# laurentbartholdi/SpaSM.jl

Measured on AMD Instinct MI355X. Metric: Schur nnz reduced/sec (GF(p) echelonize), 1Mx1M CSR, higher is better.
Workload: dtype int32 (GF(p) balanced residues); 1 GPU; BASELINE config 3: 1000000x1000000 CSR, 20 nnz/row, p=65521, seed 0x5A5A0003, Schur round 0; rows_per_gpu=1000000, npiv=169473, nnz_out=522630694, parallelism=single GPU

## Files before the change

spasm.jl_amd/csrc/engine.hip:

```cpp
#include "common.hpp"
#include "kernels.hpp"
#include "stream.hpp"
#include "wlevel.hpp"
#include "greedy.hpp"
#include "dense.hpp"
#include "spmv.hpp"
#include "spgemm.hpp"
#include "trsolve.hpp"
#include "batch.hpp"
#include <cstring>
#include <rocprim/device/device_scan.hpp>
#include <rocprim/device/device_radix_sort.hpp>
#include <vector>
#include <memory>
#include <stdexcept>
#include <type_traits>
#include <algorithm>
#include <cstring>
#include <cstdlib>
#include <condition_variable>
#include <mutex>
#include <thread>
#include <atomic>
#include <string>
// ... 94 lines not shown
}

template <int LOGT, int TPR, int WPB, int MAXR, bool SMALL, int MINW = 1> void init_scatter(size_t lds)
{
    static bool attr_done[kMaxDev] = {false};
    bool &done = attr_done[current_device()];
    if (!done) {
        HIPCHK(hipFuncSetAttribute((const void *)k_scatter<LOGT, TPR, WPB, MAXR, SMALL, MINW>, hipFuncAttributeMaxDynamicSharedMemorySize, (int)lds));
        done = true;
    }
}
template <int LOGT, int TPR, int WPB, int MAXR, bool SMALL, int MINW = 1> void launch_scatter(const ScatterArgs &a, int grid, size_t lds, hipStream_t s)
{
    init_scatter<LOGT, TPR, WPB, MAXR, SMALL, MINW>(lds);
    if (grid <= 0) return;
    hipLaunchKernelGGL((k_scatter<LOGT, TPR, WPB, MAXR, SMALL, MINW>), dim3(grid), dim3(WPB * 64), lds, s, a);
    HIPCHK(hipGetLastError());
}

template <bool SMALL> void launch_scatter_class(int cls, const ScatterArgs &a, int grid, size_t lds, hipStream_t s)
{
    switch (cls) {
    case 0: launch_scatter<8, 64, 4, 1, SMALL>(a, grid, lds, s); break;
    case 1: launch_scatter<9, 64, 4, 2, SMALL>(a, grid, lds, s); break;
    case 2: launch_scatter<10, 64, 4, 4, SMALL, 4>(a, grid, lds, s); break;
    case 3: launch_scatter<11, 128, 2, 4, SMALL, 4>(a, grid, lds, s); break;
    case 4: launch_scatter<12, 256, 4, 4, SMALL, 4>(a, grid, lds, s); break;
    case 5: launch_scatter<13, 256, 4, 5, SMALL>(a, grid, lds, s); break;
    case 6: if (SMALL) launch_scatter<14, 256, 4, 5, true>(a, grid, lds, s); break;
    default: break;
    }
}

template <int LOGT, int TPR, int WPB, int B, bool SMALL, int MINW = 1, int EPL = 1, int QX = 0, bool BLOOM = false> void launch_wstream(const StreamArgs &a, int nrows, int num_cu, size_t lds, hipStream_t s)
{
    static int per_cu_dev[kMaxDev] = {0};
    int &per_cu = per_cu_dev[current_device()];
    if (!per_cu) {
        HIPCHK(hipFuncSetAttribute((const void *)k_wstream<LOGT, TPR, WPB, B, SMALL, MINW, EPL, QX, BLOOM>, hipFuncAttributeMaxDynamicSharedMemorySize, (int)lds));
        int nb = 0;
        HIPCHK(hipOccupancyMaxActiveBlocksPerMultiprocessor(&nb, (const void *)k_wstream<LOGT, TPR, WPB, B, SMALL, MINW, EPL, QX, BLOOM>, WPB * 64, lds));
        per_cu = std::max(nb, 1);
    }
    if (nrows <= 0) return;
    const int rows_per_block = TPR == 64 ? WPB : 1;
    const int grid = std::max(1, std::min((nrows + rows_per_block - 1) / rows_per_block, num_cu * per_cu));
    hipLaunchKernelGGL((k_wstream<LOGT, TPR, WPB, B, SMALL, MINW, EPL, QX, BLOOM>), dim3(grid), dim3(WPB * 64), lds, s, a);
    HIPCHK(hipGetLastError());
}

inline bool stream_bloom()
{
    const char *e = getenv("SPASM_AMD_BLOOM");
    return e && atoi(e) != 0;
}
inline int stream_chunk_log()
{
    const char *e = getenv("SPASM_AMD_CHUNK");
    return e && atoi(e) == 128 ? 7 : 6;
}

const int kNumStreamClasses = 7;
inline int stream_logt(int c) { return 8 + c; }
inline int stream_tpr(int c) { return c <= 2 ? 64 : (c == 3 ? 128 : 256); }
inline int stream_wpb(int c) { return c == 3 ? 2 : 4; }
template <bool SMALL> void launch_stream_class(int cls, const StreamArgs &a, int nrows, int num_cu, size_t lds, hipStream_t s, int chunk_log = 6)
{
    if (chunk_log == 7) {
        switch (cls) {
        case 0: launch_wstream<8, 64, 4, 2, SMALL, 1, 2>(a, nrows, num_cu, lds, s); break;
        case 1: launch_wstream<9, 64, 4, 4, SMALL, 1, 2>(a, nrows, num_cu, lds, s); break;
        case 2: launch_wstream<10, 64, 4, 4, SMALL, 1, 2>(a, nrows, num_cu, lds, s); break;
        case 3: launch_wstream<11, 128, 2, 4, SMALL, 1, 2>(a, nrows, num_cu, lds, s); break;
        case 4: launch_wstream<12, 256, 4, 4, SMALL, 1, 2>(a, nrows, num_cu, lds, s); break;
        case 5: launch_wstream<13, 256, 4, 4, SMALL, 1, 2>(a, nrows, num_cu, lds, s); break;
        case 6: launch_wstream<14, 256, 4, 4, SMALL, 1, 2>(a, nrows, num_cu, lds, s); break;
        default: break;
        }
        return;
    }
    if (stream_bloom()) {
        switch (cls) {
        case 0: launch_wstream<8, 64, 4, 4, SMALL, 1, 1, 0, true>(a, nrows, num_cu, lds, s); break;
        case 1: launch_wstream<9, 64, 4, 8, SMALL, 1, 1, 0, true>(a, nrows, num_cu, lds, s); break;
        case 2: launch_wstream<10, 64, 4, 8, SMALL, 1, 1, 0, true>(a, nrows, num_cu, lds, s); break;
        case 3: launch_wstream<11, 128, 2, 8, SMALL, 1, 1, 0, true>(a, nrows, num_cu, lds, s); break;
        case 4: launch_wstream<12, 256, 4, 8, SMALL, 1, 1, 0, true>(a, nrows, num_cu, lds, s); break;
        case 5: launch_wstream<13, 256, 4, 8, SMALL, 1, 1, 0, true>(a, nrows, num_cu, lds, s); break;
        case 6: launch_wstream<14, 256, 4, 8, SMALL, 1, 1, 0, true>(a, nrows, num_cu, lds, s); break;
        default: break;
        }
        return;
    }
    switch (cls) {
    case 0: launch_wstream<8, 64, 4, 4, SMALL>(a, nrows, num_cu, lds, s); break;
    case 1: launch_wstream<9, 64, 4, 8, SMALL>(a, nrows, num_cu, lds, s); break;
    case 2: launch_wstream<10, 64, 4, 8, SMALL>(a, nrows, num_cu, lds, s); break;
    case 3: launch_wstream<11, 128, 2, 8, SMALL>(a, nrows, num_cu, lds, s); break;
    case 4: launch_wstream<12, 256, 4, 8, SMALL>(a, nrows, num_cu, lds, s); break;
    case 5: launch_wstream<13, 256, 4, 8, SMALL>(a, nrows, num_cu, lds, s); break;
    case 6: launch_wstream<14, 256, 4, 8, SMALL>(a, nrows, num_cu, lds, s); break;
    default: break;
    }
}

struct Round {
    ZpField F;
    int m = 0;
    int num_cu = 256;
    hipStream_t stream = nullptr;
    Scanner scan;

    DevBuf<u64d> best;
    DevBuf<int> colflag, colscan, qinv_r, pivrow, pivcol, is_piv, rowflag, rowscan, np_rows;
    int npiv = 0, nnp = 0;
    DevBuf<i64d> ulen, uoff;
    i64 utotal = 0;
    DevBuf<int2> Ufull, UPP, UPN;
    DevBuf<UHdr> uhdr;
    bool use_uinv = false;
    DevMat E;
    DevBuf<int2> UinvPool;
    DevBuf<i64d> UinvStart, ubound;
    DevBuf<int> UinvLen;
    DevBuf<int4> colinfo;
    DevBuf<unsigned> pbits;
    DevBuf<i64d> rstart;
    DevBuf<int> rlen;
    i64 uinv_nnz = 0;
    DevBuf<int4> Lpool;
    DevBuf<int> Lidx;
    bool want_idx = false;
    DevBuf<int> sflag;
    DevBuf<int2> fixbuf;
    DevBuf<int> fixcnt;
    bool use_stream = true;
    int chunk_log = 6;
    bool use_w = false;
    bool force_lists = false;
    DevBuf<int4> wcol;
    DevBuf<int2> wrow;
    DevBuf<int> wreject_list;
    i64 wtotal = 0;
    i64 wcap = 0;
    i64 w_entries = 0, w_long_rows = 0;
    i64 own_base = 0, wbase = 0;
    i64 own_total = 0;
    DevBuf<u64d> own_ctr;
    DevBuf<u64d> wstate, wblk;
    DevBuf<int> wmid_list, wbig_list, wbig_count;
    std::vector<int> wbig_at;
    bool want_w_row_stats = false;
    DevBuf<WLevRec> lev_recs;
    DevBuf<unsigned> lev0_sz, lev0_off;
    DevBuf<u64d> lev0_ent;
    i64 lev0_total = 0, lev0_entries = 0;
    int wave_per_cu_blocks = 0;
    DevBuf<int> lev, lev_keys, lev_iota, lev_order, lev_start_d, lev_flag;
    DevBuf<unsigned char> sort_tmp;
    std::vector<int> lev_start;
    int depth = -1;
    bool quiet_rejects = false;
    DevBuf<u64d> pool_ctr;
    int npool_active = NPOOL;
    u64d region_cap = 0;
    DevBuf<i64d> Lstart, bound, sstart;
    DevBuf<int> Llen, overflow_list, overflow2_list, fail_list;
    DevBuf<long long> pmask;
    int big_blocks = 0, big_npiv = -1;
    DevBuf<int> xdense;
// ... 835 lines not shown
        rstart.ensure((size_t)nrows + 1);
        rlen.ensure((size_t)nrows + 1);
        hipLaunchKernelGGL(k_gather_rows, dim3(cdiv(nrows, 256)), dim3(256), 0, stream, nrows, rows, M.start.p, M.len.p, rstart.p, rlen.p);
        HIPCHK(hipGetLastError());
        if (wmode) {
            wreject_list.ensure((size_t)nrows + 1);
            WPlanArgs wp;
            wp.nrows = nrows;
            wp.rstart = rstart.p;
            wp.rlen = rlen.p;
            wp.ent = M.ent.p;
            wp.pbits = pbits.p;
            wp.wcol = wcol.p;
            wp.Lpool = Lpool.p;
            wp.lpool_cap = region_cap;
            wp.pool_ctr = pool_ctr.p;
            wp.npool = npool_active;
            wp.upn = UPN.p;
            wp.own_base = (unsigned)own_base;
            wp.own_cap = (u64d)own_total / (u64d)npool_active;
            wp.own_ctr = own_ctr.p;
            wp.Lstart = Lstart.p;
            wp.Llen = Llen.p;
            wp.bound = bound.p;
            wp.pmask = pmask.p;
            wp.sflag = sflag.p;
            wp.free_cols = free_cols;
            wp.max_bound = (int)kClasses[kNumStreamClasses - 1].cap;
            wp.wave_row_bound = (int)kClasses[2].cap;
            wp.overflow_list = wreject_list.p;
            wp.overflow_count = &ctr.p->wplan_reject;
            wp.ctr = ctr.p;
            wp.F = F;
            chunk_log = stream_chunk_log();
            wp.chunk_log = chunk_log;
            constexpr int TEAM = 16, TPB = 256;
            hipLaunchKernelGGL((k_wplan<TEAM, TPB>), dim3(std::min(cdiv((i64)nrows * TEAM, TPB), num_cu * 16)), dim3(TPB), 0, stream, wp);
            HIPCHK(hipGetLastError());
            if (!use_uinv) {
                if (!quiet_rejects) launch_chain(a, nrows, true, wreject_list.p, &ctr.p->wplan_reject);
                return;
            }
        }
        CombineArgs c;
        c.nrows = nrows;
        c.self_idx = self_idx;
        c.rstart = rstart.p;
        c.rlen = rlen.p;
        c.ent = M.ent.p;
        c.colinfo = colinfo.p;
        c.pbits = pbits.p;
        c.uhdr = uhdr.p;
        c.UinvPool = UinvPool.p;
        c.Lpool = Lpool.p;
        c.Lidx = want_idx ? Lidx.p : nullptr;
        c.sflag = nullptr;
        c.lpool_cap = region_cap;
        c.pool_ctr = pool_ctr.p;
        c.npool = npool_active;
        c.Lstart = Lstart.p;
        c.Llen = Llen.p;
        c.bound = bound.p;
        c.pmask = pmask.p;
        c.free_cols = free_cols;
        c.retry = wmode ? wreject_list.p : nullptr;
        c.retry_count = wmode ? &ctr.p->wplan_reject : nullptr;
        c.overflow_list = overflow2_list.p;
        c.overflow_count = &ctr.p->combine_overflow;
        c.ctr = ctr.p;
        {
// ... 110 lines not shown
                HIPCHK(hipStreamCreateWithFlags(&twin_s[t], hipStreamNonBlocking));
                HIPCHK(hipEventCreateWithFlags(&twin_ev[t], hipEventDisableTiming));
            }
    }
    void ensure_big_scatter(hipStream_t s)
    {
        if (bigsc_m == m) return;
        const i64 per = std::max<i64>((i64)m, 1) * 13;
        bigsc_blocks = (int)std::max<i64>(1, std::min<i64>((i64)num_cu * 8, ((i64)2 << 30) / per));
        bigsc_m = m;
        const size_t nw = ((size_t)std::max(m, 1) + 31) / 32;
        sc_xdense.alloc((size_t)bigsc_blocks * (size_t)std::max(m, 1));
        sc_bitmap.alloc((size_t)bigsc_blocks * nw);
        sc_touched.alloc((size_t)bigsc_blocks * (size_t)std::max(m, 1));
        sc_xdense.zero(s);
        sc_bitmap.zero(s);
    }
    void warm_scatter()
    {
        ensure_streams();
        ensure_big_scatter(stream);
        ScatterArgs a;
        memset(&a, 0, sizeof a);
        StreamArgs sa;
        memset(&sa, 0, sizeof sa);
        const int nhash = F.small ? kNumHashClasses : kNumHashClasses - 1;
        for (int c = 0; c < nhash; c++) {
            const size_t lds = scatter_lds_bytes(kClasses[c], F.small);
            if (F.small) launch_scatter_class<true>(c, a, 0, lds, stream);
            else launch_scatter_class<false>(c, a, 0, lds, stream);
        }
        for (int c = 0; c < std::min(nhash, kNumStreamClasses); c++) {
            const size_t lds = stream_lds_bytes(stream_logt(c), stream_tpr(c), stream_wpb(c));
            if (F.small) launch_stream_class<true>(c, sa, 0, num_cu, lds, stream, stream_chunk_log());
            else launch_stream_class<false>(c, sa, 0, num_cu, lds, stream, stream_chunk_log());
        }
    }

    void run_scatter(const DevMat &M, const int *rows, int nrows)
    {
        const int4 *recs = Lpool.p;
        S.n = nrows;
        S.m = m;
        nlaunch = 0;
        if (nrows == 0) return;
        int nhash = F.small ? kNumHashClasses : kNumHashClasses - 1;
        const bool streaming = use_w && !force_lists && !want_idx;
        BinArgs b;
        b.nrows = nrows;
        b.bound = bound.p;
        b.Llen = Llen.p;
        for (int c = 0; c < NCLASS; c++) b.cap[c] = -1;
        for (int c = 0; c < nhash; c++) b.cap[c] = kClasses[c].cap;
        b.lazy_terms = zp_lazy_terms(F);
        b.class_count = class_count.p;
        b.class_list = class_list.p;
        b.rows = rows;
        b.start = M.start.p;
        b.len = M.len.p;
        b.orig = M.orig.p;
        b.Lstart = Lstart.p;
        b.sstart = sstart.p;
        b.pmask = pmask.p;
        b.sflag = sflag.p;
        b.stream_classes = streaming ? std::min(nhash, kNumStreamClasses) : 0;
        b.Sorig = S.orig.p;
        b.fixcnt = fixcnt.p;
        b.desc = class_desc.p;
// ... 40 lines not shown
        const bool use_side = !class_timing && (nhash > first_side || streaming);
        if (use_side) {
            ensure_streams();
            HIPCHK(hipEventRecord(ev_fork, stream));
            HIPCHK(hipStreamWaitEvent(side, ev_fork, 0));
        }
        auto mark = [&](int cls_id, hipStream_t s) {
            if (!class_timing || nlaunch >= NCLASS) return;
            HIPCHK(hipEventRecord(ev_cls[nlaunch], s));
            launch_cls[nlaunch++] = cls_id;
        };
        auto launch_class = [&](int c, hipStream_t s) {
            mark(c, s);
            a.cls = c;
            a.class_count = class_count.p + c;
            a.desc = class_desc.p + (size_t)c * nrows;
            const size_t lds = scatter_lds_bytes(kClasses[c], F.small);
            int per_cu = (int)std::min<size_t>(32 / kClasses[c].wpb, (160 * 1024) / lds);
            if (per_cu < 1) per_cu = 1;
            const int rows_per_block = kClasses[c].tpr == 64 ? kClasses[c].wpb : 1;
            const int grid = std::max(1, std::min(cdiv(nrows, rows_per_block), num_cu * per_cu));
            if (F.small) launch_scatter_class<true>(c, a, grid, lds, s);
            else launch_scatter_class<false>(c, a, grid, lds, s);
        };
        auto launch_stream_cls = [&](int c, hipStream_t s) {
            if (!streaming || c >= kNumStreamClasses) return;
            mark(NSTREAM0 + c, s);
            sa.cls = NSTREAM0 + c;
            sa.class_count = class_count.p + NSTREAM0 + c;
            sa.desc = class_desc.p + (size_t)(NSTREAM0 + c) * nrows;
            sa.redo_count = class_count.p + c;
            sa.redo_desc = class_desc.p + (size_t)c * nrows;
            const size_t lds = stream_lds_bytes(stream_logt(c), stream_tpr(c), stream_wpb(c));
            if (F.small) launch_stream_class<true>(c, sa, nrows, num_cu, lds, s, chunk_log);
            else launch_stream_class<false>(c, sa, nrows, num_cu, lds, s, chunk_log);
        };
        auto launch_stream_fix = [&](hipStream_t s) {
            if (!streaming) return;
            mark(NCLASS - 1, s);
            StreamFixArgs fa;
            fa.nrows = nrows;
            fa.fixcnt = fixcnt.p;
            fa.fixbuf = fixbuf.p;
            fa.sstart = sstart.p;
            fa.Sent = S.ent.p;
            fa.Slen = S.len.p;
            fa.Slead = S.lead.p;
            fa.ctr = ctr.p;
            fa.F = F;
            hipLaunchKernelGGL(k_stream_fix, dim3(cdiv(nrows, 64)), dim3(256), 0, s, fa);
            HIPCHK(hipGetLastError());
        };
        auto launch_big = [&](hipStream_t s) {
            ensure_big_scatter(s);
            mark(NHASHMAX - 1, s);
            BigScatterArgs bb;
            bb.s = a;
            bb.s.cls = NHASHMAX - 1;
            bb.s.class_count = class_count.p + (NHASHMAX - 1);
            bb.s.desc = class_desc.p + (size_t)(NHASHMAX - 1) * nrows;
            bb.m = std::max(m, 1);
            bb.nwords = (std::max(m, 1) + 31) / 32;
            bb.xdense = sc_xdense.p;
            bb.bitmap = sc_bitmap.p;
            bb.touched = sc_touched.p;
            hipLaunchKernelGGL(k_scatter_big, dim3(bigsc_blocks), dim3(256), 0, s, bb);
            HIPCHK(hipGetLastError());
        };
// ... 5716 lines not shown
```

spasm.jl_amd/csrc/stream.hpp:

```cpp
#pragma once
#include "kernels.hpp"

struct StreamArgs {
    const int *class_count;
    const RowDesc *desc;
    const int2 *ent;
    const int *qinv_r;
    const int2 *UPN;
    const int4 *Lpool;
    int2 *Sent;
    int *Slen;
    int *Slead;
    RoundCounters *ctr;
    int cls;
    int *redo_count;
    RowDesc *redo_desc;
    int2 *fixbuf;
    int *fixcnt;
    u64d *stamps;
    int dbg;
    ZpField F;
};

constexpr int SLCAP = 64;
// ... 186 lines not shown
}


struct WPlanArgs {
    int nrows;
    const i64d *rstart;
    const int *rlen;
    const int2 *ent;
    const unsigned *pbits;
    const int4 *wcol;
    int4 *Lpool;
    u64d lpool_cap;
    u64d *pool_ctr;
    int npool;
    int2 *upn;
    unsigned own_base;
    u64d own_cap;
    u64d *own_ctr;
    i64d *Lstart;
    int *Llen;
    i64d *bound;
    long long *pmask;
    int *sflag;
    int free_cols;
    int max_bound;
    int wave_row_bound;
    int *overflow_list;
    int *overflow_count;
    RoundCounters *ctr;
    ZpField F;
    int chunk_log;
};

template <int TEAM, int TPB>
__global__ __launch_bounds__(TPB) void k_wplan(WPlanArgs a)
{
    constexpr int TEAMS = TPB / TEAM;
    constexpr u64d RBLK = 64, OBLK = 256;
    const int tl = threadIdx.x % TEAM;
    const int team = threadIdx.x / TEAM;
    const ZpField F = a.F;
    const int CL = a.chunk_log, CH = 1 << CL;
    u64d rpos = 0, rend = 0, opos = 0, oend = 0;
    auto take = [&](u64d &pos, u64d &end, u64d need, u64d blk, u64d *ctr, u64d cap) -> u64d {
        if (pos + need > end) {
            const u64d n = need > blk ? need : blk;
            u64d b = 0;
            if (tl == 0) b = pool_alloc(ctr, cap, n, a.npool);
            b = __shfl(b, 0, TEAM);
            if (b == ~0ull) return ~0ull;
            pos = b;
            end = b + n;
        }
        const u64d r = pos;
        pos += need;
        return r;
    };
    auto is_piv = [&](int c) -> bool { return (a.pbits[(unsigned)c >> 5] >> (c & 31)) & 1u; };
    const i64d first = (i64d)blockIdx.x * TEAMS + team, stride = (i64d)gridDim.x * TEAMS;
    i64d st_n = 0;
    int ln_n = 0;
    int2 ea_n = make_int2(0, 0), eb_n = make_int2(0, 0);
    if (first < a.nrows) {
        st_n = a.rstart[first];
        ln_n = a.rlen[first];
        if (tl < ln_n) ea_n = a.ent[st_n + tl];
        if (tl + TEAM < ln_n) eb_n = a.ent[st_n + tl + TEAM];
    }
    for (i64d t64 = first; t64 < a.nrows; t64 += stride) {
        const int t = (int)t64;
        const i64d st = st_n;
        const int ln = ln_n;
        const int2 ea = ea_n, eb = eb_n;
        if (t64 + stride < a.nrows) {
            st_n = a.rstart[t64 + stride];
            ln_n = a.rlen[t64 + stride];
            ea_n = make_int2(0, 0);
            eb_n = make_int2(0, 0);
            if (tl < ln_n) ea_n = a.ent[st_n + tl];
            if (tl + TEAM < ln_n) eb_n = a.ent[st_n + tl + TEAM];
        }
        int C = 0, nN = 0;
        bool zero_own = false;
        u64d pm = 0;
        int4 ci_a = make_int4(-1, 0, 0, 0), ci_b = ci_a;
        bool pa = false, pb = false;
        for (int k0 = 0; k0 < ln; k0 += TEAM) {
            const int k = k0 + tl;
            const bool valid = k < ln;
            int2 e = k0 == 0 ? ea : (k0 == TEAM ? eb : make_int2(0, 0));
            if (k0 >= 2 * TEAM && valid) e = a.ent[st + k];
            const bool isP = valid && is_piv(e.x);
            int4 ci = make_int4(-1, 0, 0, 0);
            if (isP) ci = a.wcol[e.x];
            if (k0 == 0) { ci_a = ci; pa = isP; }
            if (k0 == TEAM) { ci_b = ci; pb = isP; }
            zero_own |= valid && (e.y == 0 || (isP && ci.y < 0));
            const u64d mP = team_ballot<TEAM>(isP);
            if (k0 < 64) pm |= mP << (k0 & 63);
            int tot;
            (void)team_incl_scan<TEAM>(isP ? (ci.y + CH - 1) >> CL : 0, tot);
            C += tot;
            nN += __popcll(team_ballot<TEAM>(valid && !isP));
        }
        const bool anyzero = team_ballot<TEAM>(zero_own) != 0;
        const int own_chunks = (nN + CH - 1) >> CL;
        const int R = C + own_chunks;
        const u64d base = take(rpos, rend, (u64d)R, RBLK, a.pool_ctr, a.lpool_cap);
        const u64d obase = base == ~0ull ? ~0ull : take(opos, oend, (u64d)nN, OBLK, a.own_ctr, a.own_cap);
        i64d run = nN;
        int w = own_chunks, no = 0;
        const bool room = base != ~0ull && obase != ~0ull;
        for (int k0 = 0; k0 < ln && room; k0 += TEAM) {
            const int k = k0 + tl;
            const bool valid = k < ln;
            int2 e = k0 == 0 ? ea : (k0 == TEAM ? eb : make_int2(0, 0));
            if (k0 >= 2 * TEAM && valid) e = a.ent[st + k];
            bool isP = k0 == 0 ? pa : (k0 == TEAM ? pb : false);
            int4 ci = k0 == 0 ? ci_a : (k0 == TEAM ? ci_b : make_int4(-1, 0, 0, 0));
            if (k0 >= 2 * TEAM) {
                isP = valid && is_piv(e.x);
                if (isP) ci = a.wcol[e.x];
            }
            const u64d mN = team_ballot<TEAM>(valid && !isP);
            if (valid && !isP) a.upn[(size_t)a.own_base + obase + no + __popcll(mN & ((1ull << tl) - 1ull))] = e;
            no += __popcll(mN);
            const int len = isP ? ci.y : 0;
            const int nch = (len + CH - 1) >> CL;
            int tot, ctot;
            const int incl = team_incl_scan<TEAM>(len, tot);
            const int cincl = team_incl_scan<TEAM>(nch, ctot);
            const int nm = zp_neg(F, e.y);
            i64d pre = run + incl - len;
            int4 *out = a.Lpool + base + w + (cincl - nch);
            for (int q = 0; q < nch; q++) {
                const int clen = min(CH, len - CH * q);
                const unsigned px = (pre < 0x8000 ? (unsigned)pre : 0x7fffu) << 16 | (unsigned)clen;
                out[q] = make_int4((int)px, nm, (int)((unsigned)ci.z + (unsigned)CH * (unsigned)q), clen);
                pre += clen;
            }
            w += ctot;
            run += tot;
        }
        if (room)
            for (int q = tl; q < own_chunks; q += TEAM) {
                const int clen = min(CH, nN - CH * q);
                a.Lpool[base + q] = make_int4((int)(((unsigned)(CH * q) << 16) | (unsigned)clen), -1, (int)(a.own_base + (unsigned)obase + (unsigned)CH * (unsigned)q), clen);
            }
        if (tl == 0) {
            if (base == ~0ull) {
                atomicAdd(&ctr_shard(a.ctr)->lpool_overflow, 1);
                a.Llen[t] = 0; a.Lstart[t] = 0; a.bound[t] = 0;
            } else {
                const i64d bound = run;
                const bool ok = room && bound <= (i64d)a.free_cols && bound <= (i64d)a.max_bound && !anyzero && R <= (bound <= (i64d)a.wave_row_bound ? 64 : 256);
                if (ok) {
                    a.Lstart[t] = (i64d)base;
                    a.Llen[t] = R;
                    a.bound[t] = bound;
                    a.pmask[t] = ln <= 32 ? (long long)pm : -1;
                    a.sflag[t] = 1;
                } else {
                    a.Llen[t] = -1; a.Lstart[t] = 0; a.bound[t] = 0;
                    a.overflow_list[atomicAdd(a.overflow_count, 1)] = t;
                }
            }
        }
    }
}

typedef int v4i32s __attribute__((ext_vector_type(4)));
template <int LOGT, int TPR, int WPB, int D, bool SMALL, int MINW, int EPL = 1, int QX = 0, bool BLOOM = false>
__global__ __launch_bounds__(WPB * 64, MINW) void k_wstream(StreamArgs a)
{
    static_assert(EPL == 1 || EPL == 2, "one or two entries per lane");
    static_assert(!(BLOOM && EPL == 2), "the filter is built for one entry per lane");
    constexpr bool WAVE_ROW = (TPR == 64);
    static_assert(WAVE_ROW || TPR == WPB * 64, "a row is owned by one wave or by the whole workgroup");
    constexpr int NW = WAVE_ROW ? 1 : WPB;
    constexpr int FCAP = SFIX;
    constexpr size_t TABB = (size_t)4 * StreamTabs<LOGT>::WORDS, MISCB = 64, FIXB = (size_t)FCAP * 8;
    constexpr size_t SLOT = stream_row_bytes(LOGT);
    extern __shared__ __attribute__((aligned(16))) unsigned char s_raw[];
    const int tid = threadIdx.x;
    const int lane = tid & 63;
    const int wave = __builtin_amdgcn_readfirstlane(tid >> 6);
    const int rtid = WAVE_ROW ? lane : tid;
    const int rw = WAVE_ROW ? 0 : wave;
    unsigned char *base = s_raw + (WAVE_ROW ? (size_t)wave * SLOT : 0);
    StreamTabs<LOGT> tb;
    tb.bind(base);
    int *misc = (int *)(base + TABB);
    int2 *fix = (int2 *)(base + TABB + MISCB);
    int4 *lst = (int4 *)(base + TABB + MISCB + FIXB);
    const ZpField F = a.F;

    const int count = *a.class_count;
    if ((WAVE_ROW ? (int)blockIdx.x * WPB : (int)blockIdx.x) >= count) return;
    for (int s = rtid * 4; s < StreamTabs<LOGT>::WORDS; s += TPR * 4) *(int4 *)(tb.t1 + s) = make_int4(0, 0, 0, 0);
    if (rtid < 16) misc[rtid] = (rtid & 7) >= 4 ? INT_MAX : 0;
    __syncthreads();

    const int first = WAVE_ROW ? (int)blockIdx.x * WPB + wave : (int)blockIdx.x;
    const int stride = WAVE_ROW ? (int)gridDim.x * WPB : (int)gridDim.x;
    u64d c_nnz = 0, c_ent = 0, c_seg = 0;
    int c_rows = 0, c_redo = 0;
    int par = 0;

    RowDesc d, dn, dnn;
    int4 rec, rec_n;
    auto load_rec = [&](const RowDesc &dd) { return a.Lpool[dd.l_start + min(rw + lane * NW, max(dd.llen - 1, 0))]; };
    d = stream_desc_unpack(stream_desc_load(a.desc + min(first, count - 1)));
    dn = stream_desc_unpack(stream_desc_load(a.desc + min(first + stride, count - 1)));
    dnn = stream_desc_unpack(stream_desc_load(a.desc + min(first + 2 * stride, count - 1)));
    rec = load_rec(d);
    rec_n = load_rec(dn);
    typedef typename std::conditional<EPL == 2, int4, int2>::type ring_t;
    ring_t ring[D];
    auto ring_load = [&](unsigned off, int clen) -> ring_t {
        if constexpr (EPL == 2) {
            const v4i32s v = *(const v4i32s *)(a.UPN + (size_t)off + (unsigned)min(2 * lane, clen - 1));
            return make_int4(v.x, v.y, v.z, v.w);
        } else {
            return a.UPN[(size_t)off + (unsigned)min(lane, clen - 1)];
        }
    };
    auto request = [&](const int4 &rc, int nmine, bool live) {
#pragma unroll
        for (int j = 0; j < D; j++) {
            const int g = min(j, max(nmine - 1, 0));
            const bool have = live && nmine > 0;
            const unsigned off = have ? (unsigned)__builtin_amdgcn_readlane(rc.z, g) : 0u;
            const int clen = have ? __builtin_amdgcn_readlane(rc.w, g) : 1;
            if constexpr (EPL == 1) {
                if (SCATTER_DBG(a, 8)) { ring[j] = make_int2(lane + 4096 * j, 1); continue; }
            }
            ring[j] = ring_load(off, clen);
        }
    };
    auto chunks_of = [&](int ll) { return ll > rw ? (ll - rw + NW - 1) / NW : 0; };
    request(rec, chunks_of(d.llen), first < count);

#ifdef SPASM_STAMPS
    u64d st_sum[NSTAMP] = {0, 0, 0, 0, 0, 0, 0, 0};
    u64d st_last = stamp_now();
#endif
    for (int w = first; w < count; w += stride) {
        const int d3_reg = stream_desc_load(a.desc + min(w + 3 * stride, count - 1));
        const int4 rec_nn = load_rec(dnn);
        const int ll = d.llen, E = d.bound, t_cur = d.t;
        int *const mrow = misc + par * 8;
        unsigned char *const rowp = (unsigned char *)(a.Sent + d.s_start);
        int mylead = INT_MAX;
        const int my_chunks = chunks_of(ll);
        STAMP(0);
        constexpr int Q = QX ? QX : (EPL == 2 ? (D >= 2 ? 2 : 1) : (D >= 4 ? 4 : D));
        constexpr int NE = Q * EPL;
        static_assert(D % Q == 0, "whole groups of slots");
        auto do_group = [&](const ring_t (&e)[Q], int g0, int nthere) {
            int cc[NE], vv[NE], pp[NE], cl[Q];
            bool there[NE];
            unsigned oo[NE], left[NE];
#pragma unroll
            for (int q = 0; q < Q; q++) {
                const int g = min(g0 + q, max(my_chunks - 1, 0));
                const int rx = __builtin_amdgcn_readlane(rec.x, g);
                const int nmul = -__builtin_amdgcn_readlane(rec.y, g);
                cl[q] = rx & 0xffff;
                if constexpr (EPL == 2) {
                    const int i0 = min(2 * lane, cl[q] - 1);
                    const bool second = 2 * lane + 1 < cl[q];
                    cc[2 * q] = e[q].x;
                    vv[2 * q] = stream_mul<SMALL>(F, nmul, e[q].y);
                    pp[2 * q] = (int)((unsigned)rx >> 16) + i0 + 1;
                    cc[2 * q + 1] = second ? e[q].z : e[q].x;
                    vv[2 * q + 1] = second ? stream_mul<SMALL>(F, nmul, e[q].w) : vv[2 * q];
                    pp[2 * q + 1] = pp[2 * q] + (second ? 1 : 0);
                    there[2 * q] = 2 * lane < cl[q];
                    there[2 * q + 1] = second;
                } else {
                    cc[q] = e[q].x;
                    vv[q] = stream_mul<SMALL>(F, nmul, e[q].y);
                    pp[q] = (int)((unsigned)rx >> 16) + min(lane, cl[q] - 1) + 1;
                    there[q] = lane < cl[q];
                }
            }
#pragma unroll
            for (int k = 0; k < NE; k++) { oo[k] = 0; left[k] = 0; }
            auto store_chunk = [&](int q) {
                if constexpr (EPL == 2) {
                    if (cl[q] == 128) {
                        v4i32s v;
                        v.x = cc[2 * q]; v.y = vv[2 * q]; v.z = cc[2 * q + 1]; v.w = vv[2 * q + 1];
                        __builtin_nontemporal_store(v, (v4i32s *)(rowp + ((unsigned)(pp[2 * q] - 1) << 3)));
                    } else {
                        __builtin_nontemporal_store(((long long)(unsigned)vv[2 * q] << 32) | (unsigned)cc[2 * q], (long long *)(rowp + ((unsigned)(pp[2 * q] - 1) << 3)));
                        __builtin_nontemporal_store(((long long)(unsigned)vv[2 * q + 1] << 32) | (unsigned)cc[2 * q + 1], (long long *)(rowp + ((unsigned)(pp[2 * q + 1] - 1) << 3)));
                    }
// ... 30 lines not shown
                }
                return;
            }
            if (nthere >= Q) {
#pragma unroll
                for (int q = 0; q < Q; q++)
                    if (!SCATTER_DBG(a, 1)) store_chunk(q);
                    else if constexpr (EPL == 2) mylead = min(mylead, min(cc[2 * q], cc[2 * q + 1]));
                    else mylead = min(mylead, cc[q]);
                if (!SCATTER_DBG(a, 2)) stream_insert_n<LOGT, NE>(tb, cc, pp, oo, left);
            } else {
#pragma unroll
                for (int q = 0; q < Q; q++)
                    if (q < nthere) {
                        store_chunk(q);
                        int c1[EPL], p1[EPL];
                        unsigned o1[EPL], l1[EPL];
#pragma unroll
                        for (int u = 0; u < EPL; u++) { c1[u] = cc[EPL * q + u]; p1[u] = pp[EPL * q + u]; }
                        stream_insert_n<LOGT, EPL>(tb, c1, p1, o1, l1);
#pragma unroll
                        for (int u = 0; u < EPL; u++) { oo[EPL * q + u] = o1[u]; left[EPL * q + u] = l1[u]; }
                    }
            }
            unsigned any = 0;
#pragma unroll
            for (int k = 0; k < NE; k++) any |= left[k];
            if (__ballot(any != 0) != 0) {
#pragma unroll
                for (int k = 0; k < NE; k++)
                    stream_report(stream_outcome(left[k]), oo[k], k / EPL < nthere && there[k], cc[k], vv[k], pp[k], mrow, fix, FCAP, lst);
            }
        };
        const int next_chunks = chunks_of(dn.llen);
        const bool next_live = w + stride < count;
#pragma unroll
        for (int j0 = 0; j0 < D; j0 += Q) {
            if (j0 < my_chunks) {
                ring_t e[Q];
#pragma unroll
                for (int q = 0; q < Q; q++) e[q] = ring[j0 + q];
                do_group(e, j0, my_chunks - j0);
            }
        }
        if (my_chunks > D) {
            for (int g0 = D; g0 < my_chunks; g0 += Q) {
                ring_t e[Q];
#pragma unroll
                for (int q = 0; q < Q; q++) {
                    const int g = min(g0 + q, my_chunks - 1);
                    e[q] = ring_load((unsigned)__builtin_amdgcn_readlane(rec.z, g), __builtin_amdgcn_readlane(rec.w, g));
                }
                do_group(e, g0, my_chunks - g0);
            }
        }
        STAMP(1);
        request(rec_n, next_chunks, next_live);
        STAMP(2);
        mylead = wave_min_i32(mylead);
        int lead_out = mylead;
        if (!WAVE_ROW) {
            if (lane == 0) mrow[4 + wave] = mylead;
            lds_barrier();
#pragma unroll
            for (int w2 = 0; w2 < WPB; w2++) lead_out = min(lead_out, mrow[4 + w2]);
        }
        if constexpr (BLOOM) {
            const int nsus = __builtin_amdgcn_readfirstlane(((lds_vint *)mrow)[1]);
            if (nsus != 0 && nsus <= SLCAP) {
                auto scan = [&](bool owners) {
                    for (int g0 = 0; g0 < my_chunks; g0 += 8) {
                        int2 e[8];
                        int ps[8], nm[8];
                        bool ok[8];
#pragma unroll
                        for (int u = 0; u < 8; u++) {
                            const int g = min(g0 + u, my_chunks - 1);
                            const int clen = __builtin_amdgcn_readlane(rec.w, g);
                            e[u] = a.UPN[(size_t)(unsigned)__builtin_amdgcn_readlane(rec.z, g) + (unsigned)min(lane, clen - 1)];
                            ps[u] = (int)((unsigned)__builtin_amdgcn_readlane(rec.x, g) >> 16) + lane;
                            nm[u] = -__builtin_amdgcn_readlane(rec.y, g);
                            ok[u] = g0 + u < my_chunks && lane < clen;
                        }
                        for (int i = 0; i < nsus; i++) {
                            const int4 sp = lst[i];
                            if (owners && !(sp.w != INT_MAX && sp.w > sp.z)) continue;
#pragma unroll
                            for (int u = 0; u < 8; u++) {
                                if (ok[u] && e[u].x == sp.x && ps[u] != sp.z) {
                                    if (!owners) atomicMin(&lst[i].w, ps[u]);
// ... 27 lines not shown
            const int nlist = __builtin_amdgcn_readfirstlane(((lds_vint *)mrow)[1]);
            redo = nlist > SLCAP;
            if (!BLOOM && nlist != 0 && !redo) {
                for (int b = 0; b < nlist; b += 64) {
                    const int i = b + lane;
                    int4 me = make_int4(-1, 0, -1, 0);
                    if (i < nlist) me = lst[i];
                    int owner = -1;
                    for (int j = 0; j < nlist; j++) {
                        const int4 o = lst[j];
                        if (j < i && owner < 0 && o.x == me.x && o.z != me.z) owner = o.z;
                    }
                    if (owner >= 0) stream_fix_push(mrow, fix, FCAP, owner, me.z, me.y);
                }
            }
            const int nfix = SCATTER_DBG(a, 4) ? 0 : __builtin_amdgcn_readfirstlane(((lds_vint *)mrow)[0]);
            redo = redo || nfix > FCAP;
            if (redo) {
                if (lane == 0) {
                    const int at = atomicAdd(a.redo_count, 1);
                    a.redo_desc[at] = d;
                }
                c_redo += 1;
            } else {
                if (lane < nfix) a.fixbuf[(size_t)t_cur * SFIX + lane] = fix[lane];
                if (lane == 0) {
                    a.Slen[t_cur] = E;
                    a.Slead[t_cur] = E > 0 ? lead_out : INT_MAX;
                    if (nfix) a.fixcnt[t_cur] = nfix;
                }
                c_nnz += (u64d)E;
                c_rows += E > 0;
                c_ent += (u64d)E;
                c_seg += 1 + (u64d)ll;
            }
        }
        STAMP(3);
        for (int s = rtid * 4; s < StreamTabs<LOGT>::WORDS; s += TPR * 4) *(int4 *)(tb.t1 + s) = make_int4(0, 0, 0, 0);
        if (WAVE_ROW) {
            if (lane < 2) mrow[lane] = 0;
            __builtin_amdgcn_wave_barrier();
        } else {
            par ^= 1;
            if (rtid < 8) misc[par * 8 + rtid] = rtid >= 4 ? INT_MAX : 0;
            lds_barrier();
        }
        STAMP(4);
        d = dn;
        dn = dnn;
        dnn = stream_desc_unpack(d3_reg);
        rec = rec_n; rec_n = rec_nn;
        STAMP(5);
    }
#ifdef SPASM_STAMPS
    if (lane == 0 && a.stamps) {
        for (int i = 0; i < NSTAMP; i++) atomicAdd(&a.stamps[(size_t)a.cls * 2 * NSTAMP + i], st_sum[i]);
        atomicAdd(&a.stamps[(size_t)a.cls * 2 * NSTAMP + NSTAMP], 1ull);
    }
#endif
    if (lane == 0 && (WAVE_ROW || wave == 0)) {
        if (c_nnz) atomicAdd(&ctr_shard(a.ctr)->nnz_out, c_nnz);
        if (c_rows) atomicAdd(&ctr_shard(a.ctr)->nonempty_out, c_rows);
        if (c_redo) atomicAdd(&ctr_shard(a.ctr)->stream_redo, c_redo);
        if (c_ent | c_seg) {
            atomicAdd(&ctr_shard(a.ctr)->class_ent[a.cls], c_ent);
            atomicAdd(&ctr_shard(a.ctr)->class_seg[a.cls], c_seg);
        }
// ... 48 lines not shown
```

Measured before the change: 170.0 billion nnz/s.

## Add segment-based streaming mode that locates entries by position instead of chunks

Adds a SEG stream mode, the default when the buffer is under 2^29 entries. The planner writes one Lpool record per pivot segment instead of one per 64-entry chunk. The stream kernel then finds each lane's source segment with ballots over segment start positions and loads entries directly. This cuts planning work, record count and the wasted lanes in partially filled chunks, at the cost of per-chunk segment lookup loops. It also rejects rows with more than 64 segments.

```diff
diff --git a/spasm.jl_amd/csrc/engine.hip b/spasm.jl_amd/csrc/engine.hip
--- a/spasm.jl_amd/csrc/engine.hip
+++ b/spasm.jl_amd/csrc/engine.hip
@@ -150,20 +150,20 @@
     }
 }
 
-template <int LOGT, int TPR, int WPB, int B, bool SMALL, int MINW = 1, int EPL = 1, int QX = 0, bool BLOOM = false> void launch_wstream(const StreamArgs &a, int nrows, int num_cu, size_t lds, hipStream_t s)
+template <int LOGT, int TPR, int WPB, int B, bool SMALL, int MINW = 1, int EPL = 1, int QX = 0, bool BLOOM = false, bool SEG = false> void launch_wstream(const StreamArgs &a, int nrows, int num_cu, size_t lds, hipStream_t s)
 {
     static int per_cu_dev[kMaxDev] = {0};
     int &per_cu = per_cu_dev[current_device()];
     if (!per_cu) {
-        HIPCHK(hipFuncSetAttribute((const void *)k_wstream<LOGT, TPR, WPB, B, SMALL, MINW, EPL, QX, BLOOM>, hipFuncAttributeMaxDynamicSharedMemorySize, (int)lds));
+        HIPCHK(hipFuncSetAttribute((const void *)k_wstream<LOGT, TPR, WPB, B, SMALL, MINW, EPL, QX, BLOOM, SEG>, hipFuncAttributeMaxDynamicSharedMemorySize, (int)lds));
         int nb = 0;
-        HIPCHK(hipOccupancyMaxActiveBlocksPerMultiprocessor(&nb, (const void *)k_wstream<LOGT, TPR, WPB, B, SMALL, MINW, EPL, QX, BLOOM>, WPB * 64, lds));
+        HIPCHK(hipOccupancyMaxActiveBlocksPerMultiprocessor(&nb, (const void *)k_wstream<LOGT, TPR, WPB, B, SMALL, MINW, EPL, QX, BLOOM, SEG>, WPB * 64, lds));
         per_cu = std::max(nb, 1);
     }
     if (nrows <= 0) return;
     const int rows_per_block = TPR == 64 ? WPB : 1;
     const int grid = std::max(1, std::min((nrows + rows_per_block - 1) / rows_per_block, num_cu * per_cu));
-    hipLaunchKernelGGL((k_wstream<LOGT, TPR, WPB, B, SMALL, MINW, EPL, QX, BLOOM>), dim3(grid), dim3(WPB * 64), lds, s, a);
+    hipLaunchKernelGGL((k_wstream<LOGT, TPR, WPB, B, SMALL, MINW, EPL, QX, BLOOM, SEG>), dim3(grid), dim3(WPB * 64), lds, s, a);
     HIPCHK(hipGetLastError());
 }
 
@@ -176,15 +176,35 @@
 {
     const char *e = getenv("SPASM_AMD_CHUNK");
     return e && atoi(e) == 128 ? 7 : 6;
+}
+enum StreamMode { STREAM_SEG = 0, STREAM_CHUNK64 = 1, STREAM_BLOOM = 2, STREAM_CHUNK128 = 3 };
+inline StreamMode stream_mode(i64 buffer_entries)
+{
+    if (stream_chunk_log() == 7) return STREAM_CHUNK128;
+    if (stream_bloom()) return STREAM_BLOOM;
+    return buffer_entries < ((i64)1 << 29) ? STREAM_SEG : STREAM_CHUNK64;
 }
 
 const int kNumStreamClasses = 7;
 inline int stream_logt(int c) { return 8 + c; }
 inline int stream_tpr(int c) { return c <= 2 ? 64 : (c == 3 ? 128 : 256); }
 inline int stream_wpb(int c) { return c == 3 ? 2 : 4; }
-template <bool SMALL> void launch_stream_class(int cls, const StreamArgs &a, int nrows, int num_cu, size_t lds, hipStream_t s, int chunk_log = 6)
-{
-    if (chunk_log == 7) {
+template <bool SMALL> void launch_stream_class(int cls, const StreamArgs &a, int nrows, int num_cu, size_t lds, hipStream_t s, StreamMode mode)
+{
+    if (mode == STREAM_SEG) {
+        switch (cls) {
+        case 0: launch_wstream<8, 64, 4, 4, SMALL, 1, 1, 0, false, true>(a, nrows, num_cu, lds, s); break;
+        case 1: launch_wstream<9, 64, 4, 8, SMALL, 1, 1, 0, false, true>(a, nrows, num_cu, lds, s); break;
+        case 2: launch_wstream<10, 64, 4, 8, SMALL, 1, 1, 0, false, true>(a, nrows, num_cu, lds, s); break;
+        case 3: launch_wstream<11, 128, 2, 8, SMALL, 1, 1, 0, false, true>(a, nrows, num_cu, lds, s); break;
+        case 4: launch_wstream<12, 256, 4, 8, SMALL, 1, 1, 0, false, true>(a, nrows, num_cu, lds, s); break;
+        case 5: launch_wstream<13, 256, 4, 8, SMALL, 1, 1, 0, false, true>(a, nrows, num_cu, lds, s); break;
+        case 6: launch_wstream<14, 256, 4, 8, SMALL, 1, 1, 0, false, true>(a, nrows, num_cu, lds, s); break;
+        default: break;
+        }
+        return;
+    }
+    if (mode == STREAM_CHUNK128) {
         switch (cls) {
         case 0: launch_wstream<8, 64, 4, 2, SMALL, 1, 2>(a, nrows, num_cu, lds, s); break;
         case 1: launch_wstream<9, 64, 4, 4, SMALL, 1, 2>(a, nrows, num_cu, lds, s); break;
@@ -197,7 +217,7 @@
         }
         return;
     }
-    if (stream_bloom()) {
+    if (mode == STREAM_BLOOM) {
         switch (cls) {
         case 0: launch_wstream<8, 64, 4, 4, SMALL, 1, 1, 0, true>(a, nrows, num_cu, lds, s); break;
         case 1: launch_wstream<9, 64, 4, 8, SMALL, 1, 1, 0, true>(a, nrows, num_cu, lds, s); break;
@@ -253,7 +273,7 @@
     DevBuf<int2> fixbuf;
     DevBuf<int> fixcnt;
     bool use_stream = true;
-    int chunk_log = 6;
+    StreamMode smode = STREAM_SEG;
     bool use_w = false;
     bool force_lists = false;
     DevBuf<int4> wcol;
@@ -1155,10 +1175,12 @@
             wp.overflow_count = &ctr.p->wplan_reject;
             wp.ctr = ctr.p;
             wp.F = F;
-            chunk_log = stream_chunk_log();
-            wp.chunk_log = chunk_log;
+            smode = stream_mode(wbase + wcap);
+            wp.chunk_log = smode == STREAM_CHUNK128 ? 7 : 6;
             constexpr int TEAM = 16, TPB = 256;
-            hipLaunchKernelGGL((k_wplan<TEAM, TPB>), dim3(std::min(cdiv((i64)nrows * TEAM, TPB), num_cu * 16)), dim3(TPB), 0, stream, wp);
+            const dim3 grid(std::min(cdiv((i64)nrows * TEAM, TPB), num_cu * 16));
+            if (smode == STREAM_SEG) hipLaunchKernelGGL((k_wplan<TEAM, TPB, true>), grid, dim3(TPB), 0, stream, wp);
+            else hipLaunchKernelGGL((k_wplan<TEAM, TPB, false>), grid, dim3(TPB), 0, stream, wp);
             HIPCHK(hipGetLastError());
             if (!use_uinv) {
                 if (!quiet_rejects) launch_chain(a, nrows, true, wreject_list.p, &ctr.p->wplan_reject);
@@ -1335,8 +1357,9 @@
         }
         for (int c = 0; c < std::min(nhash, kNumStreamClasses); c++) {
             const size_t lds = stream_lds_bytes(stream_logt(c), stream_tpr(c), stream_wpb(c));
-            if (F.small) launch_stream_class<true>(c, sa, 0, num_cu, lds, stream, stream_chunk_log());
-            else launch_stream_class<false>(c, sa, 0, num_cu, lds, stream, stream_chunk_log());
+            const StreamMode mode = stream_mode(use_w ? wbase + wcap : 0);
+            if (F.small) launch_stream_class<true>(c, sa, 0, num_cu, lds, stream, mode);
+            else launch_stream_class<false>(c, sa, 0, num_cu, lds, stream, mode);
         }
     }
 
@@ -1443,8 +1466,8 @@
             sa.redo_count = class_count.p + c;
             sa.redo_desc = class_desc.p + (size_t)c * nrows;
             const size_t lds = stream_lds_bytes(stream_logt(c), stream_tpr(c), stream_wpb(c));
-            if (F.small) launch_stream_class<true>(c, sa, nrows, num_cu, lds, s, chunk_log);
-            else launch_stream_class<false>(c, sa, nrows, num_cu, lds, s, chunk_log);
+            if (F.small) launch_stream_class<true>(c, sa, nrows, num_cu, lds, s, smode);
+            else launch_stream_class<false>(c, sa, nrows, num_cu, lds, s, smode);
         };
         auto launch_stream_fix = [&](hipStream_t s) {
             if (!streaming) return;
diff --git a/spasm.jl_amd/csrc/stream.hpp b/spasm.jl_amd/csrc/stream.hpp
--- a/spasm.jl_amd/csrc/stream.hpp
+++ b/spasm.jl_amd/csrc/stream.hpp
@@ -242,7 +242,7 @@
     int chunk_log;
 };
 
-template <int TEAM, int TPB>
+template <int TEAM, int TPB, bool SEGP>
 __global__ __launch_bounds__(TPB) void k_wplan(WPlanArgs a)
 {
     constexpr int TEAMS = TPB / TEAM;
@@ -308,20 +308,24 @@
             zero_own |= valid && (e.y == 0 || (isP && ci.y < 0));
             const u64d mP = team_ballot<TEAM>(isP);
             if (k0 < 64) pm |= mP << (k0 & 63);
-            int tot;
-            (void)team_incl_scan<TEAM>(isP ? (ci.y + CH - 1) >> CL : 0, tot);
-            C += tot;
+            if constexpr (SEGP) C += __popcll(mP);
+            else {
+                int tot;
+                (void)team_incl_scan<TEAM>(isP ? (ci.y + CH - 1) >> CL : 0, tot);
+                C += tot;
+            }
             nN += __popcll(team_ballot<TEAM>(valid && !isP));
         }
         const bool anyzero = team_ballot<TEAM>(zero_own) != 0;
-        const int own_chunks = (nN + CH - 1) >> CL;
+        const int own_chunks = SEGP ? (nN > 0 ? 1 : 0) : (nN + CH - 1) >> CL;
         const int R = C + own_chunks;
-        const u64d base = take(rpos, rend, (u64d)R, RBLK, a.pool_ctr, a.lpool_cap);
-        const u64d obase = base == ~0ull ? ~0ull : take(opos, oend, (u64d)nN, OBLK, a.own_ctr, a.own_cap);
+        const bool fits = !SEGP || R <= 64;
+        const u64d base = take(rpos, rend, fits ? (u64d)R : 0, RBLK, a.pool_ctr, a.lpool_cap);
+        const u64d obase = base == ~0ull ? ~0ull : take(opos, oend, fits ? (u64d)nN : 0, OBLK, a.own_ctr, a.own_cap);
         i64d run = nN;
         int w = own_chunks, no = 0;
         const bool room = base != ~0ull && obase != ~0ull;
-        for (int k0 = 0; k0 < ln && room; k0 += TEAM) {
+        for (int k0 = 0; k0 < ln && room && fits; k0 += TEAM) {
             const int k = k0 + tl;
             const bool valid = k < ln;
             int2 e = k0 == 0 ? ea : (k0 == TEAM ? eb : make_int2(0, 0));
@@ -336,34 +340,47 @@
             if (valid && !isP) a.upn[(size_t)a.own_base + obase + no + __popcll(mN & ((1ull << tl) - 1ull))] = e;
             no += __popcll(mN);
             const int len = isP ? ci.y : 0;
-            const int nch = (len + CH - 1) >> CL;
-            int tot, ctot;
+            int tot;
             const int incl = team_incl_scan<TEAM>(len, tot);
-            const int cincl = team_incl_scan<TEAM>(nch, ctot);
             const int nm = zp_neg(F, e.y);
             i64d pre = run + incl - len;
-            int4 *out = a.Lpool + base + w + (cincl - nch);
-            for (int q = 0; q < nch; q++) {
-                const int clen = min(CH, len - CH * q);
-                const unsigned px = (pre < 0x8000 ? (unsigned)pre : 0x7fffu) << 16 | (unsigned)clen;
-                out[q] = make_int4((int)px, nm, (int)((unsigned)ci.z + (unsigned)CH * (unsigned)q), clen);
-                pre += clen;
-            }
-            w += ctot;
+            if constexpr (SEGP) {
+                const u64d mP = team_ballot<TEAM>(isP);
+                const unsigned px = (pre < 0x8000 ? (unsigned)pre : 0x7fffu) << 16 | (unsigned)min(len, 0xffff);
+                if (isP) a.Lpool[base + w + __popcll(mP & ((1ull << tl) - 1ull))] = make_int4((int)px, nm, ci.z, len);
+                w += __popcll(mP);
+            } else {
+                const int nch = (len + CH - 1) >> CL;
+                int ctot;
+                const int cincl = team_incl_scan<TEAM>(nch, ctot);
+                int4 *out = a.Lpool + base + w + (cincl - nch);
+                for (int q = 0; q < nch; q++) {
+                    const int clen = min(CH, len - CH * q);
+                    const unsigned px = (pre < 0x8000 ? (unsigned)pre : 0x7fffu) << 16 | (unsigned)clen;
+                    out[q] = make_int4((int)px, nm, (int)((unsigned)ci.z + (unsigned)CH * (unsigned)q), clen);
+                    pre += clen;
+                }
+                w += ctot;
+            }
             run += tot;
         }
-        if (room)
-            for (int q = tl; q < own_chunks; q += TEAM) {
-                const int clen = min(CH, nN - CH * q);
-                a.Lpool[base + q] = make_int4((int)(((unsigned)(CH * q) << 16) | (unsigned)clen), -1, (int)(a.own_base + (unsigned)obase + (unsigned)CH * (unsigned)q), clen);
-            }
+        if (room && fits) {
+            if constexpr (SEGP) {
+                if (tl == 0 && nN > 0) a.Lpool[base] = make_int4(min(nN, 0xffff), -1, (int)(a.own_base + (unsigned)obase), nN);
+            } else {
+                for (int q = tl; q < own_chunks; q += TEAM) {
+                    const int clen = min(CH, nN - CH * q);
+                    a.Lpool[base + q] = make_int4((int)(((unsigned)(CH * q) << 16) | (unsigned)clen), -1, (int)(a.own_base + (unsigned)obase + (unsigned)CH * (unsigned)q), clen);
+                }
+            }
+        }
         if (tl == 0) {
             if (base == ~0ull) {
                 atomicAdd(&ctr_shard(a.ctr)->lpool_overflow, 1);
                 a.Llen[t] = 0; a.Lstart[t] = 0; a.bound[t] = 0;
             } else {
                 const i64d bound = run;
-                const bool ok = room && bound <= (i64d)a.free_cols && bound <= (i64d)a.max_bound && !anyzero && R <= (bound <= (i64d)a.wave_row_bound ? 64 : 256);
+                const bool ok = room && fits && bound <= (i64d)a.free_cols && bound <= (i64d)a.max_bound && !anyzero && R <= (SEGP || bound <= (i64d)a.wave_row_bound ? 64 : 256);
                 if (ok) {
                     a.Lstart[t] = (i64d)base;
                     a.Llen[t] = R;
@@ -380,11 +397,12 @@
 }
 
 typedef int v4i32s __attribute__((ext_vector_type(4)));
-template <int LOGT, int TPR, int WPB, int D, bool SMALL, int MINW, int EPL = 1, int QX = 0, bool BLOOM = false>
+template <int LOGT, int TPR, int WPB, int D, bool SMALL, int MINW, int EPL = 1, int QX = 0, bool BLOOM = false, bool SEG = false>
 __global__ __launch_bounds__(WPB * 64, MINW) void k_wstream(StreamArgs a)
 {
     static_assert(EPL == 1 || EPL == 2, "one or two entries per lane");
     static_assert(!(BLOOM && EPL == 2), "the filter is built for one entry per lane");
+    static_assert(!SEG || (EPL == 1 && !BLOOM), "the cut by position is built for one entry per lane and the exact tables");
     constexpr bool WAVE_ROW = (TPR == 64);
     static_assert(WAVE_ROW || TPR == WPB * 64, "a row is owned by one wave or by the whole workgroup");
     constexpr int NW = WAVE_ROW ? 1 : WPB;
@@ -419,7 +437,7 @@
 
     RowDesc d, dn, dnn;
     int4 rec, rec_n;
-    auto load_rec = [&](const RowDesc &dd) { return a.Lpool[dd.l_start + min(rw + lane * NW, max(dd.llen - 1, 0))]; };
+    auto load_rec = [&](const RowDesc &dd) { return a.Lpool[dd.l_start + min(SEG ? lane : rw + lane * NW, max(dd.llen - 1, 0))]; };
     d = stream_desc_unpack(stream_desc_load(a.desc + min(first, count - 1)));
     dn = stream_desc_unpack(stream_desc_load(a.desc + min(first + stride, count - 1)));
     dnn = stream_desc_unpack(stream_desc_load(a.desc + min(first + 2 * stride, count - 1)));
@@ -427,6 +445,32 @@
     rec_n = load_rec(dn);
     typedef typename std::conditional<EPL == 2, int4, int2>::type ring_t;
     ring_t ring[D];
+    int rmul[D];
+    struct SegRegs { int st, dl, nm; };
+    auto seg_regs = [&](const int4 &rc, int nseg) {
+        SegRegs r;
+        const int st = (int)((unsigned)rc.x >> 16);
+        r.st = lane < nseg ? st : INT_MAX;
+        r.dl = rc.z - st;
+        r.nm = -rc.y;
+        return r;
+    };
+    auto seg_locate = [&](const SegRegs &r, int E, int g, unsigned &boff, int &mu) {
+        const int p0 = (rw + g * NW) << 6;
+        const int pos = min(p0 + lane, E - 1);
+        const int n1 = __popcll(__ballot(r.st <= p0));
+        const int n2 = __popcll(__ballot(r.st <= p0 + 63));
+        const int cur = max(n1 - 1, 0);
+        int dl = __builtin_amdgcn_readlane(r.dl, cur);
+        mu = __builtin_amdgcn_readlane(r.nm, cur);
+        for (int s = n1; s < n2; s++) {
+            const bool in = pos >= __builtin_amdgcn_readlane(r.st, s);
+            dl = in ? __builtin_amdgcn_readlane(r.dl, s) : dl;
+            mu = in ? __builtin_amdgcn_readlane(r.nm, s) : mu;
+        }
+        boff = (unsigned)(pos + dl) << 3;
+    };
+    auto seg_load = [&](unsigned boff) { return *(const int2 *)((const unsigned char *)a.UPN + boff); };
     auto ring_load = [&](unsigned off, int clen) -> ring_t {
         if constexpr (EPL == 2) {
             const v4i32s v = *(const v4i32s *)(a.UPN + (size_t)off + (unsigned)min(2 * lane, clen - 1));
@@ -435,7 +479,20 @@
             return a.UPN[(size_t)off + (unsigned)min(lane, clen - 1)];
         }
     };
-    auto request = [&](const int4 &rc, int nmine, bool live) {
+    auto request = [&](const int4 &rc, int nmine, bool live, int nseg, int E) {
+        if constexpr (SEG) {
+            const SegRegs r = seg_regs(rc, nseg);
+            unsigned boff = 0;
+            int mu = 0;
+#pragma unroll
+            for (int j = 0; j < D; j++) {
+                if (live && j < nmine) seg_locate(r, E, j, boff, mu);
+                asm volatile("" : "+v"(boff));
+                ring[j] = seg_load(boff);
+                rmul[j] = mu;
+            }
+            return;
+        }
 #pragma unroll
         for (int j = 0; j < D; j++) {
             const int g = min(j, max(nmine - 1, 0));
@@ -449,7 +506,8 @@
         }
     };
     auto chunks_of = [&](int ll) { return ll > rw ? (ll - rw + NW - 1) / NW : 0; };
-    request(rec, chunks_of(d.llen), first < count);
+    auto row_chunks = [&](const RowDesc &dd) { return SEG ? (dd.bound + 63) >> 6 : dd.llen; };
+    request(rec, chunks_of(row_chunks(d)), first < count, d.llen, d.bound);
 
 #ifdef SPASM_STAMPS
     u64d st_sum[NSTAMP] = {0, 0, 0, 0, 0, 0, 0, 0};
@@ -462,18 +520,27 @@
         int *const mrow = misc + par * 8;
         unsigned char *const rowp = (unsigned char *)(a.Sent + d.s_start);
         int mylead = INT_MAX;
-        const int my_chunks = chunks_of(ll);
+        const int my_chunks = chunks_of(row_chunks(d));
         STAMP(0);
         constexpr int Q = QX ? QX : (EPL == 2 ? (D >= 2 ? 2 : 1) : (D >= 4 ? 4 : D));
         constexpr int NE = Q * EPL;
         static_assert(D % Q == 0, "whole groups of slots");
-        auto do_group = [&](const ring_t (&e)[Q], int g0, int nthere) {
+        auto do_group = [&](const ring_t (&e)[Q], const int (&emul)[Q], int g0, int nthere) {
             int cc[NE], vv[NE], pp[NE], cl[Q];
             bool there[NE];
             unsigned oo[NE], left[NE];
 #pragma unroll
             for (int q = 0; q < Q; q++) {
                 const int g = min(g0 + q, max(my_chunks - 1, 0));
+                if constexpr (SEG) {
+                    const int p0 = (rw + g * NW) << 6;
+                    cl[q] = 64;
+                    cc[q] = e[q].x;
+                    vv[q] = stream_mul<SMALL>(F, emul[q], e[q].y);
+                    pp[q] = min(p0 + lane, E - 1) + 1;
+                    there[q] = p0 + lane < E;
+                    continue;
+                }
                 const int rx = __builtin_amdgcn_readlane(rec.x, g);
                 const int nmul = -__builtin_amdgcn_readlane(rec.y, g);
                 cl[q] = rx & 0xffff;
@@ -570,30 +637,41 @@
                     stream_report(stream_outcome(left[k]), oo[k], k / EPL < nthere && there[k], cc[k], vv[k], pp[k], mrow, fix, FCAP, lst);
             }
         };
-        const int next_chunks = chunks_of(dn.llen);
+        const int next_chunks = chunks_of(row_chunks(dn));
         const bool next_live = w + stride < count;
 #pragma unroll
         for (int j0 = 0; j0 < D; j0 += Q) {
             if (j0 < my_chunks) {
                 ring_t e[Q];
-#pragma unroll
-                for (int q = 0; q < Q; q++) e[q] = ring[j0 + q];
-                do_group(e, j0, my_chunks - j0);
+                int em[Q];
+#pragma unroll
+                for (int q = 0; q < Q; q++) { e[q] = ring[j0 + q]; em[q] = SEG ? rmul[j0 + q] : 0; }
+                do_group(e, em, j0, my_chunks - j0);
             }
         }
         if (my_chunks > D) {
+            SegRegs sr = {0, 0, 0};
+            if constexpr (SEG) sr = seg_regs(rec, ll);
             for (int g0 = D; g0 < my_chunks; g0 += Q) {
                 ring_t e[Q];
+                int em[Q];
 #pragma unroll
                 for (int q = 0; q < Q; q++) {
                     const int g = min(g0 + q, my_chunks - 1);
-                    e[q] = ring_load((unsigned)__builtin_amdgcn_readlane(rec.z, g), __builtin_amdgcn_readlane(rec.w, g));
-                }
-                do_group(e, g0, my_chunks - g0);
+                    em[q] = 0;
+                    if constexpr (SEG) {
+                        unsigned boff;
+                        seg_locate(sr, E, g, boff, em[q]);
+                        e[q] = seg_load(boff);
+                    } else {
+                        e[q] = ring_load((unsigned)__builtin_amdgcn_readlane(rec.z, g), __builtin_amdgcn_readlane(rec.w, g));
+                    }
+                }
+                do_group(e, em, g0, my_chunks - g0);
             }
         }
         STAMP(1);
-        request(rec_n, next_chunks, next_live);
+        request(rec_n, next_chunks, next_live, dn.llen, dn.bound);
         STAMP(2);
         mylead = wave_min_i32(mylead);
         int lead_out = mylead;
@@ -687,7 +765,7 @@
                 c_nnz += (u64d)E;
                 c_rows += E > 0;
                 c_ent += (u64d)E;
-                c_seg += 1 + (u64d)ll;
+                c_seg += 1 + (u64d)row_chunks(d);
             }
         }
         STAMP(3);
```

Measured after the change: 189.1 billion nnz/s (median of 6 runs). 1.11x the previous value.
